# shenyunhang/APE

Hardware: NVIDIA H100
Metric: images_per_sec (higher is better)
Workload: dtype f16

## Files before the change

ape_b200/csrc/gemm_tc.cu:

```cuda
#include <stdlib.h>

#include <type_traits>

#include "common.cuh"
#include "tc.cuh"

namespace ape {
namespace {

constexpr int BM = 128, BK = 64, WG_K = 16;
constexpr int kConsumerWarps = 8;
constexpr int kThreads = 32 * kConsumerWarps + 32;

enum Act { ACT_NONE = 0, ACT_RELU = 1, ACT_GELU = 2, ACT_SWIGLU = 3, ACT_CLAMP = 4 };
enum Res { RES_NONE = 0, RES_F32 = 1, RES_16 = 2 };

template <bool OUT32, int ACT, int RES, bool LN = false, bool ROPE = false, bool STATS = false>
struct Epi {
  static constexpr bool out32 = OUT32, ln = LN, rope = ROPE, stats = STATS;
  static constexpr int act = ACT, res = RES;
};

struct GemmParams {
  void *C;
// ... 245 lines not shown
  if (threadIdx.x == 0) trace_stamp(p, 1);

  if (warp == kConsumerWarps) {
    if (lane == 0) {
      uint32_t stage = 0, phase = 0;
      int m_blk, n_blk;
      for (int t = 0; tile_at(t, m_blk, n_blk); ++t) {
        for (int kb = 0; kb < p.k_blocks; ++kb) {
          tc::mbar_wait(&s.empty[stage], phase ^ 1);
          tc::mbar_expect_tx(&s.full[stage], STAGE_BYTES);
          if (p.conv) {
            const int img = m_blk / p.conv_tiles_img, tt = m_blk - img * p.conv_tiles_img;
            const int ty = tt / p.conv_tiles_x, tx = tt - ty * p.conv_tiles_x;
            const int tap = kb / p.conv_cblks, cb = kb - tap * p.conv_cblks;
            tc::tma_load_4d(s.a[stage], &map_a, &s.full[stage], cb * BK, tx * p.conv_tw + tap % 3 - 1, ty * p.conv_th + tap / 3 - 1, img);
          } else {
            tc::tma_load_2d(s.a[stage], &map_a, &s.full[stage], kb * BK, m_blk * BM);
          }
          if (CL == 1) {
            tc::tma_load_2d(s.b[stage], &map_b, &s.full[stage], kb * BK, n_blk * BN);
          } else {
            constexpr int HALF_ROWS = BN / CL;
            tc::tma_load_2d_multicast(s.b[stage] + rank * HALF_ROWS * BK * 2, &map_b, &s.full[stage], kb * BK,
                                      n_blk * BN + rank * HALF_ROWS, (uint16_t)((1u << CL) - 1));
          }
          if (++stage == STAGES) { stage = 0; phase ^= 1; }
        }
      }
    }
    __syncwarp();
  } else {
    const int wg = warp / 4;
    float acc[BN / 2];
#pragma unroll
    for (int i = 0; i < BN / 2; ++i) acc[i] = 0.f;
    auto release = [&](uint32_t st) {
      if (lane == 0) {
        tc::mbar_arrive(&s.empty[st]);
        if (CL > 1) tc::mbar_arrive_cluster(tc::mapa_u32(&s.empty[st], (uint32_t)(rank ^ 1)));
      }
    };
    uint32_t stage = 0, phase = 0;
    int m_blk, n_blk;
    for (int t = 0; tile_at(t, m_blk, n_blk); ++t) {
      uint32_t prev = 0;
      for (int kb = 0; kb < p.k_blocks; ++kb) {
        tc::mbar_wait(&s.full[stage], phase);
        if (kb == 0 && t == 0 && threadIdx.x == 0) trace_stamp(p, 2);
        const uint64_t da = tc::make_smem_desc_sw128(tc::smem_u32(s.a[stage] + wg * 64 * BK * 2));
        const uint64_t db = tc::make_smem_desc_sw128(tc::smem_u32(s.b[stage]));
        tc::fence_regs<BN / 2>(acc);
        tc::wgmma_fence();
#pragma unroll
        for (int k = 0; k < BK / WG_K; ++k)
          tc::Wgmma<BN, TI>::template ss<0>(acc, da + 2 * k, db + 2 * k, (kb | k) != 0);
        tc::wgmma_commit();
        tc::fence_regs<BN / 2>(acc);
        if (kb > 0) {
          tc::wgmma_wait<1>();
          release(prev);
        }
        prev = stage;
        if (++stage == STAGES) { stage = 0; phase ^= 1; }
      }
      tc::wgmma_wait<0>();
      tc::fence_regs<BN / 2>(acc);
      release(prev);
      if (threadIdx.x == 0) {
        trace_stamp(p, 3);
        if (t == 0) trace_stamp(p, 4);
        trace_stamp(p, 5);
      }
      if constexpr (kArgmax<E>) argmax_epilogue<BN>(p, acc, m_blk, n_blk, wg, lane);
      else if (!E::rope && p.fast && (m_blk + 1) * BM <= p.M && (n_blk + 1) * BN <= p.N) epilogue<E, TI, BN, true>(p, acc, m_blk, n_blk, wg, lane);
      else epilogue<E, TI, BN, false>(p, acc, m_blk, n_blk, wg, lane);
    }
    if (threadIdx.x == 0) trace_stamp(p, 6);
  }
  __syncthreads();
  if (CL > 1) tc::cluster_sync_all();
  if (threadIdx.x == 0) trace_stamp(p, 7);
}

typedef CUresult (*EncodeTiledFn)(CUtensorMap *, CUtensorMapDataType, cuuint32_t, void *, const cuuint64_t *,
                                  const cuuint64_t *, const cuuint32_t *, const cuuint32_t *, CUtensorMapInterleave,
                                  CUtensorMapSwizzle, CUtensorMapL2promotion, CUtensorMapFloatOOBfill);

EncodeTiledFn get_encoder() {
  static EncodeTiledFn fn = nullptr;
  if (fn == nullptr) {
    void *ptr = nullptr;
    cudaDriverEntryPointQueryResult qres;
    if (cudaGetDriverEntryPoint("cuTensorMapEncodeTiled", &ptr, cudaEnableDefault, &qres) == cudaSuccess &&
        qres == cudaDriverEntryPointSuccess)
      fn = reinterpret_cast<EncodeTiledFn>(ptr);
  }
  return fn;
}

int make_map(CUtensorMap *map, const void *base, int dtype, long long rows, long long K, long long ld, int box_rows,
             int box_cols = BK) {
  EncodeTiledFn enc = get_encoder();
  if (!enc) return fail(APE_ERR_UNSUPPORTED, "gemm: cuTensorMapEncodeTiled not available from the driver");
  cuuint64_t dims[2] = {(cuuint64_t)K, (cuuint64_t)rows};
  cuuint64_t strides[1] = {(cuuint64_t)ld * (dtype == APE_DTYPE_F32 ? 4 : 2)};
  cuuint32_t box[2] = {(cuuint32_t)box_cols, (cuuint32_t)box_rows};
  cuuint32_t estr[2] = {1, 1};
  CUresult r = enc(map, dtype == APE_DTYPE_F32 ? CU_TENSOR_MAP_DATA_TYPE_FLOAT32
                        : dtype == APE_DTYPE_F16 ? CU_TENSOR_MAP_DATA_TYPE_FLOAT16 : CU_TENSOR_MAP_DATA_TYPE_BFLOAT16, 2,
                   const_cast<void *>(base), dims, strides, box, estr, CU_TENSOR_MAP_INTERLEAVE_NONE,
                   CU_TENSOR_MAP_SWIZZLE_128B, CU_TENSOR_MAP_L2_PROMOTION_L2_256B, CU_TENSOR_MAP_FLOAT_OOB_FILL_NONE);
  if (r != CUDA_SUCCESS) return fail(APE_ERR_INVALID_ARG, "gemm: cuTensorMapEncodeTiled failed (%d)", (int)r);
  return APE_OK;
}

int num_sms() {
  static int n = 0;
  if (n == 0) {
    int dev = 0;
    cudaGetDevice(&dev);
    cudaDeviceGetAttribute(&n, cudaDevAttrMultiProcessorCount, dev);
    if (n <= 0) n = 132;
  }
  return n;
}

template <int BN, int STAGES, int CL, typename TI, class E>
int launch_gemm(const CUtensorMap &ma, const CUtensorMap &mb, GemmParams &p, cudaStream_t st) {
  using Smem = GemmSmem<BN, STAGES>;
  const size_t smem = sizeof(Smem) + 1024;
  auto k = gemm_tc_kernel<BN, STAGES, CL, TI, E>;
  static bool attr_set = false;
  if (!attr_set) {
    cudaError_t e = cudaFuncSetAttribute(k, cudaFuncAttributeMaxDynamicSharedMemorySize, (int)smem);
    if (e != cudaSuccess) return fail((int)e, "gemm: cudaFuncSetAttribute(smem=%zu): %s", smem, cudaGetErrorString(e));
    attr_set = true;
  }
  p.n_blocks = (p.N + BN - 1) / BN;
  const int m_groups = (p.m_blocks + CL - 1) / CL;
  const int groups = m_groups * p.n_blocks;
  const int max_clusters = num_sms() / CL;
  const int clusters = groups < max_clusters ? groups : max_clusters;
  p.band = std::min(m_groups, (clusters + p.n_blocks - 1) / p.n_blocks);
  cudaLaunchConfig_t cfg{};
  cfg.gridDim = dim3((unsigned)(clusters * CL));
  cfg.blockDim = dim3(kThreads);
  cfg.dynamicSmemBytes = smem;
  cfg.stream = st;
  cudaLaunchAttribute attr[2];
  attr[0].id = cudaLaunchAttributeClusterDimension;
  attr[0].val.clusterDim.x = CL;
  attr[0].val.clusterDim.y = 1;
  attr[0].val.clusterDim.z = 1;
  attr[1].id = cudaLaunchAttributeProgrammaticStreamSerialization;
  attr[1].val.programmaticStreamSerializationAllowed = pdl_enabled() ? 1 : 0;
  cfg.attrs = attr;
  cfg.numAttrs = 2;
  cudaError_t e = cudaLaunchKernelEx(&cfg, k, ma, mb, p);
  if (e != cudaSuccess) return fail((int)e, "gemm_tc_kernel launch: %s", cudaGetErrorString(e));
  return check_launch("gemm_tc_kernel");
}

template <int CL, typename TI, class E>
int launch_bn(int bn, const CUtensorMap &ma, const CUtensorMap &mb, GemmParams &p, cudaStream_t st) {
  if (bn == 256) return launch_gemm<256, 4, CL, TI, E>(ma, mb, p, st);
  return launch_gemm<128, 6, CL, TI, E>(ma, mb, p, st);
}

struct EpiKey {
  bool out32;
  int act, res;
  bool ln, rope, stats;
};

#define APE_GEMM_EPILOGUES(X)                                                                                            \
  X(false, ACT_NONE, RES_NONE, false, false, false) X(false, ACT_RELU, RES_NONE, false, false, false)                   \
  X(false, ACT_GELU, RES_NONE, false, false, false) X(false, ACT_NONE, RES_F32, false, false, false)                    \
  X(false, ACT_NONE, RES_16, false, false, false) X(false, ACT_RELU, RES_16, false, false, false)                       \
  X(false, ACT_GELU, RES_16, false, false, false) X(false, ACT_SWIGLU, RES_NONE, false, false, false)                   \
  X(false, ACT_SWIGLU, RES_NONE, false, false, true) X(false, ACT_NONE, RES_NONE, false, true, false)                   \
  X(true, ACT_NONE, RES_NONE, false, false, false) X(true, ACT_RELU, RES_NONE, false, false, false)                     \
  X(true, ACT_GELU, RES_NONE, false, false, false) X(true, ACT_SWIGLU, RES_NONE, false, false, false)                   \
  X(true, ACT_CLAMP, RES_NONE, false, false, false) X(true, ACT_NONE, RES_F32, false, false, false)                     \
  X(true, ACT_NONE, RES_16, false, false, false) X(true, ACT_NONE, RES_F32, true, false, false)

template <int CL, typename TI>
int launch_epi(int bn, const EpiKey &k, const CUtensorMap &ma, const CUtensorMap &mb, GemmParams &p, cudaStream_t st) {
#define APE_EPI_CASE(o, a, r, l, ro, s)                                                                                  \
  if (k.out32 == o && k.act == a && k.res == r && k.ln == l && k.rope == ro && k.stats == s)                           \
    return launch_bn<CL, TI, Epi<o, a, r, l, ro, s>>(bn, ma, mb, p, st);
  APE_GEMM_EPILOGUES(APE_EPI_CASE)
#undef APE_EPI_CASE
  return fail(APE_ERR_UNSUPPORTED, "gemm: no kernel for the epilogue (fp32 out %d, act %d, residual %d, ln %d, rope %d, stats %d)",
              (int)k.out32, k.act, k.res, (int)k.ln, (int)k.rope, (int)k.stats);
}

int launch_any(int bn, bool cluster, int in_dtype, const EpiKey &k, const CUtensorMap &ma, const CUtensorMap &mb, GemmParams &p,
               cudaStream_t st) {
  if (in_dtype == APE_DTYPE_BF16)
    return cluster ? launch_epi<2, __nv_bfloat16>(bn, k, ma, mb, p, st) : launch_epi<1, __nv_bfloat16>(bn, k, ma, mb, p, st);
  return cluster ? launch_epi<2, __half>(bn, k, ma, mb, p, st) : launch_epi<1, __half>(bn, k, ma, mb, p, st);
}

}
}

using namespace ape;

struct RopeArgs {
  const float *cos, *sin;
  const int *pos;
  int cols, npos;
};

struct FuseArgs {
  const float *ln_part, *ln_colsum;
  int ln_nparts;
  float ln_inv_c, ln_eps;
  float *stats_out;
  int stats_nslab;
};

static long long *g_gemm_trace = nullptr;

extern "C" void ape_gemm_set_trace(long long *device_buffer) { g_gemm_trace = device_buffer; }

static int gemm_impl(const void *A, int64_t lda, const void *W, int64_t ldw, void *C, int64_t ldc,
                     const float *bias, const void *residual, int64_t ldr, int res_dtype, int M, int N, int K, int in_dtype,
                     int out_dtype, int act, int tile_n, const RopeArgs *rope, void *stream, const FuseArgs *fuse = nullptr) {
  if (residual && res_dtype != APE_DTYPE_F32 && res_dtype != APE_DTYPE_F16 && res_dtype != APE_DTYPE_BF16)
    return fail(APE_ERR_INVALID_ARG, "gemm: bad res_dtype %d", res_dtype);
  if (in_dtype != APE_DTYPE_F16 && in_dtype != APE_DTYPE_BF16)
    return fail(APE_ERR_INVALID_ARG, "gemm: operands must be fp16 or bf16 (got dtype %d)", in_dtype);
  if (out_dtype != APE_DTYPE_F32 && out_dtype != APE_DTYPE_F16 && out_dtype != APE_DTYPE_BF16)
    return fail(APE_ERR_INVALID_ARG, "gemm: bad out_dtype %d", out_dtype);
  if (act < 0 || act > ACT_CLAMP) return fail(APE_ERR_INVALID_ARG, "gemm: bad activation %d", act);
  if (M < 0 || N <= 0 || K <= 0) return fail(APE_ERR_INVALID_ARG, "gemm: bad sizes M=%d N=%d K=%d", M, N, K);
  if (M == 0) return APE_OK;
  if (!A || !W || !C) return fail(APE_ERR_NULL_PTR, "gemm: null pointer argument");
  if ((lda * 2) % 16 || (ldw * 2) % 16 || (reinterpret_cast<uintptr_t>(A) & 15) || (reinterpret_cast<uintptr_t>(W) & 15))
    return fail(APE_ERR_INVALID_ARG, "gemm: A/W base and row pitch must be 16-byte aligned (TMA)");
  if (lda < K || ldw < K) return fail(APE_ERR_INVALID_ARG, "gemm: row pitch smaller than K");
  if (act == ACT_SWIGLU && ((N & 1) || residual)) return fail(APE_ERR_INVALID_ARG, "gemm: swiglu needs even N, no residual");
  const int bn = (tile_n & 0xfff) > 0 ? (tile_n & 0xfff) : 128;
  if (bn != 128 && bn != 256) return fail(APE_ERR_INVALID_ARG, "gemm: tile_n must be 128 or 256");
  if (tile_n & 0x2000) return fail(APE_ERR_UNSUPPORTED, "gemm: tile_n flag 0x2000 (CTA-pair MMA) is not available on sm_90a");
  cudaStream_t st = reinterpret_cast<cudaStream_t>(stream);
  const int m_blocks = (M + BM - 1) / BM;
  const bool cluster = m_blocks >= 2 && (tile_n & 0x1000) == 0 && ((tile_n & 0x4000) != 0 || K >= 2048);
  CUtensorMap ma, mb;
  if (int rc = make_map(&ma, A, in_dtype, M, K, lda, BM)) return rc;
  if (int rc = make_map(&mb, W, in_dtype, N, K, ldw, cluster ? bn / 2 : bn)) return rc;
  GemmParams p{};
  p.C = C; p.bias = bias; p.residual = residual; p.ldc = ldc; p.ldr = ldr;
  p.M = M; p.N = N; p.K = K;
  p.m_blocks = m_blocks;
  p.k_blocks = (K + BK - 1) / BK;
  p.trace = g_gemm_trace;
  const int oe = out_dtype == APE_DTYPE_F32 ? 4 : 2;
  if (oe == 2 && out_dtype != in_dtype)
    return fail(APE_ERR_UNSUPPORTED, "gemm: a 16-bit output must have the operand dtype (out %d, operands %d)", out_dtype, in_dtype);
  if (residual && res_dtype != APE_DTYPE_F32 && res_dtype != in_dtype)
    return fail(APE_ERR_UNSUPPORTED, "gemm: a 16-bit residual must have the operand dtype (residual %d, operands %d)", res_dtype, in_dtype);
  const auto pairs = [](const void *ptr, long long ld, int esize) {
    return (ld % 2) == 0 && (reinterpret_cast<uintptr_t>(ptr) % (2 * esize)) == 0;
  };
  p.vec_out = pairs(C, ldc, oe);
  p.fast = p.vec_out && (!residual || pairs(residual, ldr, res_dtype == APE_DTYPE_F32 ? 4 : 2)) &&
           reinterpret_cast<uintptr_t>(bias) % 8 == 0 && (!fuse || reinterpret_cast<uintptr_t>(fuse->ln_colsum) % 8 == 0);
  EpiKey key{oe == 4, act, !residual ? RES_NONE : res_dtype == APE_DTYPE_F32 ? RES_F32 : RES_16, false, rope != nullptr, false};
  const int n_out = act == ACT_SWIGLU ? N / 2 : N;
  if (fuse) {
    if (fuse->ln_part) {
      if (out_dtype != APE_DTYPE_F32 || !fuse->ln_colsum || fuse->ln_nparts <= 0 || act == ACT_SWIGLU)
        return fail(APE_ERR_INVALID_ARG, "gemm+ln: needs an fp32 output, column sums and partial statistics");
      p.ln_part = fuse->ln_part; p.ln_colsum = fuse->ln_colsum; p.ln_nparts = fuse->ln_nparts;
      p.ln_inv_c = fuse->ln_inv_c; p.ln_eps = fuse->ln_eps;
      key.ln = true;
    }
    if (fuse->stats_out) {
      if (oe != 2 || act != ACT_SWIGLU || fuse->stats_nslab != (n_out + 63) / 64)
        return fail(APE_ERR_INVALID_ARG, "gemm+stats: needs the SwiGLU epilogue with a 16-bit output and stats_nslab = ceil(N/2/64)");
      p.stats_out = fuse->stats_out; p.stats_nslab = fuse->stats_nslab;
      key.stats = true;
    }
  }
  if (rope) {
    if (oe != 2 || act != ACT_NONE || rope->cols % 64 != 0 || rope->cols > N || rope->npos <= 0 || !rope->cos || !rope->sin)
      return fail(APE_ERR_INVALID_ARG, "gemm+rope: needs a 16-bit output, no activation, rope_cols a multiple of 64 <= N");
    p.rope_cos = rope->cos; p.rope_sin = rope->sin; p.rope_pos = rope->pos; p.rope_cols = rope->cols; p.rope_npos = rope->npos;
  }
  return launch_any(bn, cluster, in_dtype, key, ma, mb, p, st);
}

extern "C" int ape_gemm_tn(const void *A, int64_t lda, const void *W, int64_t ldw, void *C, int64_t ldc,
                           const float *bias, const void *residual, int64_t ldr, int M, int N, int K, int in_dtype,
                           int out_dtype, int act, int tile_n, void *stream) {
  return gemm_impl(A, lda, W, ldw, C, ldc, bias, residual, ldr, out_dtype, M, N, K, in_dtype, out_dtype, act, tile_n, nullptr,
                   stream);
}

extern "C" int ape_gemm_tn_ex(const void *A, int64_t lda, const void *W, int64_t ldw, void *C, int64_t ldc,
                              const float *bias, const void *residual, int64_t ldr, int res_dtype, int M, int N, int K,
                              int in_dtype, int out_dtype, int act, int tile_n, void *stream) {
  return gemm_impl(A, lda, W, ldw, C, ldc, bias, residual, ldr, res_dtype, M, N, K, in_dtype, out_dtype, act, tile_n, nullptr,
                   stream);
}

extern "C" int ape_gemm_tn_fused(const void *A, int64_t lda, const void *W, int64_t ldw, void *C, int64_t ldc, const float *bias,
                                 const void *residual, int64_t ldr, int res_dtype, int M, int N, int K, int in_dtype, int out_dtype,
                                 int act, int tile_n, const float *ln_part, int ln_nparts, const float *ln_colsum, float ln_inv_c,
                                 float ln_eps, float *stats_out, int stats_nslab, void *stream) {
  FuseArgs f{ln_part, ln_colsum, ln_nparts, ln_inv_c, ln_eps, stats_out, stats_nslab};
  return gemm_impl(A, lda, W, ldw, C, ldc, bias, residual, ldr, res_dtype, M, N, K, in_dtype, out_dtype, act, tile_n, nullptr,
                   stream, &f);
}

static int make_map_nhwc(CUtensorMap *map, const void *base, int dtype, int B, int H, int W, int C, int bw, int bh) {
  EncodeTiledFn enc = get_encoder();
  if (!enc) return fail(APE_ERR_UNSUPPORTED, "conv: cuTensorMapEncodeTiled not available from the driver");
  cuuint64_t dims[4] = {(cuuint64_t)C, (cuuint64_t)W, (cuuint64_t)H, (cuuint64_t)B};
  cuuint64_t strides[3] = {(cuuint64_t)C * 2, (cuuint64_t)W * C * 2, (cuuint64_t)H * W * C * 2};
  cuuint32_t box[4] = {64, (cuuint32_t)bw, (cuuint32_t)bh, 1};
  cuuint32_t estr[4] = {1, 1, 1, 1};
  CUresult r = enc(map, dtype == APE_DTYPE_F16 ? CU_TENSOR_MAP_DATA_TYPE_FLOAT16 : CU_TENSOR_MAP_DATA_TYPE_BFLOAT16, 4,
                   const_cast<void *>(base), dims, strides, box, estr, CU_TENSOR_MAP_INTERLEAVE_NONE,
                   CU_TENSOR_MAP_SWIZZLE_128B, CU_TENSOR_MAP_L2_PROMOTION_L2_256B, CU_TENSOR_MAP_FLOAT_OOB_FILL_NONE);
  if (r != CUDA_SUCCESS) return fail(APE_ERR_INVALID_ARG, "conv: cuTensorMapEncodeTiled failed (%d)", (int)r);
  return APE_OK;
}

extern "C" int ape_conv3x3_nhwc(const void *x, const void *w, void *y, const float *bias, int B, int H, int W, int Cin, int Cout,
                                int dtype, int act, void *stream) {
  if (dtype != APE_DTYPE_F16 && dtype != APE_DTYPE_BF16) return fail(APE_ERR_INVALID_ARG, "conv3x3: fp16 / bf16 only");
  if (B <= 0 || H <= 0 || W <= 0 || Cin <= 0 || Cout <= 0) return fail(APE_ERR_INVALID_ARG, "conv3x3: bad sizes");
  if (Cin % 64 || Cout % 8) return fail(APE_ERR_UNSUPPORTED, "conv3x3: Cin must be a multiple of 64 and Cout of 8 (got %d, %d)", Cin, Cout);
  if (act != ACT_NONE && act != ACT_RELU && act != ACT_GELU) return fail(APE_ERR_INVALID_ARG, "conv3x3: activation %d", act);
  int tw = 128;
  while (tw > 8 && W % tw) tw >>= 1;
  const int th = 128 / tw;
  if (W % tw || H % th) return fail(APE_ERR_UNSUPPORTED, "conv3x3: %dx%d image is not a whole number of %dx%d pixel tiles", H, W, th, tw);
  if (!x || !w || !y) return fail(APE_ERR_NULL_PTR, "conv3x3: null pointer argument");
  if ((reinterpret_cast<uintptr_t>(x) | reinterpret_cast<uintptr_t>(w) | reinterpret_cast<uintptr_t>(y)) & 15)
    return fail(APE_ERR_INVALID_ARG, "conv3x3: tensors must be 16-byte aligned");
  const int K = 9 * Cin, M = B * H * W, N = Cout;
  const int bn = 128;
  const int m_blocks = M / BM;
  const bool cluster = m_blocks >= 2 && m_blocks % 2 == 0;
  CUtensorMap ma, mb;
  if (int rc = make_map_nhwc(&ma, x, dtype, B, H, W, Cin, tw, th)) return rc;
  if (int rc = make_map(&mb, w, dtype, N, K, K, cluster ? bn / 2 : bn)) return rc;
  GemmParams p{};
  p.C = y; p.bias = bias; p.ldc = N; p.M = M; p.N = N; p.K = K;
  p.m_blocks = m_blocks;
  p.k_blocks = K / BK;
  p.vec_out = 1;
  p.fast = reinterpret_cast<uintptr_t>(bias) % 8 == 0;
  p.conv = 1; p.conv_tw = tw; p.conv_th = th; p.conv_tiles_x = W / tw; p.conv_tiles_img = (W / tw) * (H / th); p.conv_cblks = Cin / 64;
  p.conv_W = W; p.conv_H = H;
  const EpiKey key{false, act, RES_NONE, false, false, false};
  return launch_any(bn, cluster, dtype, key, ma, mb, p, reinterpret_cast<cudaStream_t>(stream));
}

extern "C" int ape_gemm_tn_argmax(const void *A, int64_t lda, const void *W, int64_t ldw, uint64_t *keys, int M, int N, int K,
                                  int col_base, int in_dtype, void *stream) {
  if (in_dtype != APE_DTYPE_F16 && in_dtype != APE_DTYPE_BF16)
    return fail(APE_ERR_INVALID_ARG, "gemm_argmax: operands must be fp16 or bf16 (got dtype %d)", in_dtype);
  if (M < 0 || N <= 0 || K <= 0 || col_base < 0 || (long long)col_base + N > 0x7fffffffLL)
    return fail(APE_ERR_INVALID_ARG, "gemm_argmax: bad sizes M=%d N=%d K=%d col_base=%d", M, N, K, col_base);
  if (M == 0) return APE_OK;
  if (!A || !W || !keys) return fail(APE_ERR_NULL_PTR, "gemm_argmax: null pointer argument");
  if ((lda * 2) % 16 || (ldw * 2) % 16 || (reinterpret_cast<uintptr_t>(A) & 15) || (reinterpret_cast<uintptr_t>(W) & 15))
    return fail(APE_ERR_INVALID_ARG, "gemm_argmax: A/W base and row pitch must be 16-byte aligned (TMA)");
  if (lda < K || ldw < K) return fail(APE_ERR_INVALID_ARG, "gemm_argmax: row pitch smaller than K");
  if (reinterpret_cast<uintptr_t>(keys) & 7) return fail(APE_ERR_INVALID_ARG, "gemm_argmax: keys must be 8-byte aligned");
  constexpr int bn = 128;
  CUtensorMap ma, mb;
  if (int rc = make_map(&ma, A, in_dtype, M, K, lda, BM)) return rc;
  if (int rc = make_map(&mb, W, in_dtype, N, K, ldw, bn)) return rc;
  GemmParams p{};
  p.C = keys; p.M = M; p.N = N; p.K = K;
  p.m_blocks = (M + BM - 1) / BM;
  p.k_blocks = (K + BK - 1) / BK;
  p.trace = g_gemm_trace;
  p.argmax_col_base = col_base;
  cudaStream_t st = reinterpret_cast<cudaStream_t>(stream);
  if (in_dtype == APE_DTYPE_BF16) return launch_gemm<bn, 6, 1, __nv_bfloat16, EpiArgmax>(ma, mb, p, st);
  return launch_gemm<bn, 6, 1, __half, EpiArgmax>(ma, mb, p, st);
}

extern "C" int ape_gemm_tn_rope(const void *A, int64_t lda, const void *W, int64_t ldw, void *C, int64_t ldc,
                                const float *bias, int M, int N, int K, int in_dtype, int out_dtype, const float *cos_table,
                                const float *sin_table, const int *pos_map, int npos, int head_dim, int rope_cols,
                                int tile_n, void *stream) {
  if (head_dim != 64) return fail(APE_ERR_UNSUPPORTED, "gemm+rope: head_dim %d (only 64)", head_dim);
  if ((reinterpret_cast<uintptr_t>(cos_table) | reinterpret_cast<uintptr_t>(sin_table)) & 15)
    return fail(APE_ERR_INVALID_ARG, "gemm+rope: cos / sin tables must be 16-byte aligned");
  RopeArgs r{cos_table, sin_table, pos_map, rope_cols, npos};
  return gemm_impl(A, lda, W, ldw, C, ldc, bias, nullptr, 0, out_dtype, M, N, K, in_dtype, out_dtype, ACT_NONE, tile_n, &r, stream);
}
```

ape_b200/csrc/tc.cuh:

```cuda
#pragma once
#include <cuda.h>
#include <cuda_runtime.h>
#include <cuda_fp16.h>
#include <cuda_bf16.h>
#include <stdint.h>

namespace ape {
namespace tc {

__device__ __forceinline__ uint32_t smem_u32(const void *p) {
  return (uint32_t)__cvta_generic_to_shared(p);
}

__device__ __forceinline__ void mbar_init(uint64_t *bar, uint32_t count) {
  asm volatile("mbarrier.init.shared::cta.b64 [%0], %1;" ::"r"(smem_u32(bar)), "r"(count) : "memory");
}
__device__ __forceinline__ void fence_mbar_init() {
  asm volatile("fence.mbarrier_init.release.cluster;" ::: "memory");
}
__device__ __forceinline__ void mbar_expect_tx(uint64_t *bar, uint32_t bytes) {
  asm volatile("mbarrier.arrive.expect_tx.shared::cta.b64 _, [%0], %1;" ::"r"(smem_u32(bar)), "r"(bytes)
               : "memory");
}
__device__ __forceinline__ void mbar_arrive(uint64_t *bar) {
  asm volatile("mbarrier.arrive.shared::cta.b64 _, [%0];" ::"r"(smem_u32(bar)) : "memory");
}
__device__ __forceinline__ void mbar_wait(uint64_t *bar, uint32_t parity) {
  const uint32_t addr = smem_u32(bar);
  for (uint32_t it = 0; it < (1u << 26); ++it) {
    uint32_t done;
    asm volatile(
        "{\n\t.reg .pred p;\n\t"
        "mbarrier.try_wait.parity.shared::cta.b64 p, [%1], %2;\n\t"
        "selp.u32 %0, 1, 0, p;\n\t}"
        : "=r"(done)
        : "r"(addr), "r"(parity)
        : "memory");
    if (done) return;
  }
  __trap();
}

__device__ __forceinline__ void prefetch_tensormap(const CUtensorMap *m) {
  asm volatile("prefetch.tensormap [%0];" ::"l"(m) : "memory");
}
__device__ __forceinline__ void tma_load_2d(void *smem_dst, const CUtensorMap *map, uint64_t *bar, int c0, int c1) {
  asm volatile(
      "cp.async.bulk.tensor.2d.shared::cluster.global.tile.mbarrier::complete_tx::bytes [%0], [%1, {%3, %4}], [%2];"
      ::"r"(smem_u32(smem_dst)), "l"(map), "r"(smem_u32(bar)), "r"(c0), "r"(c1)
      : "memory");
}

__device__ __forceinline__ void tma_load_4d(void *smem_dst, const CUtensorMap *map, uint64_t *bar, int c0, int c1, int c2, int c3) {
  asm volatile(
      "cp.async.bulk.tensor.4d.shared::cluster.global.tile.mbarrier::complete_tx::bytes [%0], [%1, {%3, %4, %5, %6}], [%2];"
      ::"r"(smem_u32(smem_dst)), "l"(map), "r"(smem_u32(bar)), "r"(c0), "r"(c1), "r"(c2), "r"(c3)
      : "memory");
}

__device__ __forceinline__ void tma_load_2d_multicast(void *smem_dst, const CUtensorMap *map, uint64_t *bar, int c0,
                                                      int c1, uint16_t cta_mask) {
  asm volatile(
      "cp.async.bulk.tensor.2d.shared::cluster.global.tile.mbarrier::complete_tx::bytes.multicast::cluster"
      " [%0], [%1, {%3, %4}], [%2], %5;"
      ::"r"(smem_u32(smem_dst)), "l"(map), "r"(smem_u32(bar)), "r"(c0), "r"(c1), "h"(cta_mask)
      : "memory");
}
__device__ __forceinline__ uint32_t cluster_ctarank() {
  uint32_t r;
  asm volatile("mov.u32 %0, %%cluster_ctarank;" : "=r"(r));
  return r;
}
__device__ __forceinline__ void cluster_sync_all() {
  asm volatile("barrier.cluster.arrive.release.aligned;" ::: "memory");
  asm volatile("barrier.cluster.wait.acquire.aligned;" ::: "memory");
}

__device__ __forceinline__ uint32_t mapa_u32(const void *p, uint32_t rank) {
  uint32_t r;
  asm volatile("mapa.shared::cluster.u32 %0, %1, %2;" : "=r"(r) : "r"(smem_u32(p)), "r"(rank));
  return r;
}
__device__ __forceinline__ void mbar_arrive_cluster(uint32_t bar_cluster_addr) {
  asm volatile("mbarrier.arrive.release.cluster.shared::cluster.b64 _, [%0];" ::"r"(bar_cluster_addr) : "memory");
}

template <int N>
__device__ __forceinline__ void setmaxnreg_inc() { asm volatile("setmaxnreg.inc.sync.aligned.u32 %0;" ::"n"(N)); }
template <int N>
__device__ __forceinline__ void setmaxnreg_dec() { asm volatile("setmaxnreg.dec.sync.aligned.u32 %0;" ::"n"(N)); }

__device__ __forceinline__ void wgmma_fence() { asm volatile("wgmma.fence.sync.aligned;" ::: "memory"); }
__device__ __forceinline__ void wgmma_commit() { asm volatile("wgmma.commit_group.sync.aligned;" ::: "memory"); }
template <int N>
__device__ __forceinline__ void wgmma_wait() { asm volatile("wgmma.wait_group.sync.aligned %0;" ::"n"(N) : "memory"); }
template <int N>
__device__ __forceinline__ void fence_regs(float *r) {
#pragma unroll
  for (int i = 0; i < N; ++i) asm volatile("" : "+f"(r[i])::"memory");
}
__device__ __forceinline__ void fence_proxy_async() { asm volatile("fence.proxy.async.shared::cta;" ::: "memory"); }

__device__ __forceinline__ uint64_t make_smem_desc_sw128(uint32_t smem_addr) {
  uint64_t d = 0;
  d |= (uint64_t)((smem_addr & 0x3FFFF) >> 4);
  d |= (uint64_t)1 << 16;
  d |= (uint64_t)(1024 >> 4) << 32;
  d |= (uint64_t)1 << 62;
  return d;
}

template <int N, typename T>
struct Wgmma;
template <> struct Wgmma<64, __half> {
  template <int TRANS_B>
  __device__ static __forceinline__ void ss(float *d, uint64_t da, uint64_t db, int scale_d) {
    asm volatile(
        "{\n.reg .pred p;\nsetp.ne.b32 p, %34, 0;\n"
        "wgmma.mma_async.sync.aligned.m64n64k16.f32.f16.f16 {%0, %1, %2, %3, %4, %5, %6, %7, %8, %9, %10, %11, %12, %13, %14, %15, %16, %17, %18, %19, %20, %21, %22, %23, %24, %25, %26, %27, %28, %29, %30, %31}, %32, %33, p, 1, 1, 0, %35;\n}\n"
        : "+f"(d[0]), "+f"(d[1]), "+f"(d[2]), "+f"(d[3]), "+f"(d[4]), "+f"(d[5]), "+f"(d[6]), "+f"(d[7]), "+f"(d[8]), "+f"(d[9]), "+f"(d[10]), "+f"(d[11]), "+f"(d[12]), "+f"(d[13]), "+f"(d[14]), "+f"(d[15]), "+f"(d[16]), "+f"(d[17]), "+f"(d[18]), "+f"(d[19]), "+f"(d[20]), "+f"(d[21]), "+f"(d[22]), "+f"(d[23]), "+f"(d[24]), "+f"(d[25]), "+f"(d[26]), "+f"(d[27]), "+f"(d[28]), "+f"(d[29]), "+f"(d[30]), "+f"(d[31])
        : "l"(da), "l"(db), "r"(scale_d), "n"(TRANS_B));
  }
  template <int TRANS_B>
  __device__ static __forceinline__ void rs(float *d, const uint32_t *a, uint64_t db, int scale_d) {
    asm volatile(
        "{\n.reg .pred p;\nsetp.ne.b32 p, %37, 0;\n"
        "wgmma.mma_async.sync.aligned.m64n64k16.f32.f16.f16 {%0, %1, %2, %3, %4, %5, %6, %7, %8, %9, %10, %11, %12, %13, %14, %15, %16, %17, %18, %19, %20, %21, %22, %23, %24, %25, %26, %27, %28, %29, %30, %31}, {%32, %33, %34, %35}, %36, p, 1, 1, %38;\n}\n"
        : "+f"(d[0]), "+f"(d[1]), "+f"(d[2]), "+f"(d[3]), "+f"(d[4]), "+f"(d[5]), "+f"(d[6]), "+f"(d[7]), "+f"(d[8]), "+f"(d[9]), "+f"(d[10]), "+f"(d[11]), "+f"(d[12]), "+f"(d[13]), "+f"(d[14]), "+f"(d[15]), "+f"(d[16]), "+f"(d[17]), "+f"(d[18]), "+f"(d[19]), "+f"(d[20]), "+f"(d[21]), "+f"(d[22]), "+f"(d[23]), "+f"(d[24]), "+f"(d[25]), "+f"(d[26]), "+f"(d[27]), "+f"(d[28]), "+f"(d[29]), "+f"(d[30]), "+f"(d[31])
        : "r"(a[0]), "r"(a[1]), "r"(a[2]), "r"(a[3]), "l"(db), "r"(scale_d), "n"(TRANS_B));
  }
};
template <> struct Wgmma<64, __nv_bfloat16> {
  template <int TRANS_B>
  __device__ static __forceinline__ void ss(float *d, uint64_t da, uint64_t db, int scale_d) {
    asm volatile(
        "{\n.reg .pred p;\nsetp.ne.b32 p, %34, 0;\n"
        "wgmma.mma_async.sync.aligned.m64n64k16.f32.bf16.bf16 {%0, %1, %2, %3, %4, %5, %6, %7, %8, %9, %10, %11, %12, %13, %14, %15, %16, %17, %18, %19, %20, %21, %22, %23, %24, %25, %26, %27, %28, %29, %30, %31}, %32, %33, p, 1, 1, 0, %35;\n}\n"
        : "+f"(d[0]), "+f"(d[1]), "+f"(d[2]), "+f"(d[3]), "+f"(d[4]), "+f"(d[5]), "+f"(d[6]), "+f"(d[7]), "+f"(d[8]), "+f"(d[9]), "+f"(d[10]), "+f"(d[11]), "+f"(d[12]), "+f"(d[13]), "+f"(d[14]), "+f"(d[15]), "+f"(d[16]), "+f"(d[17]), "+f"(d[18]), "+f"(d[19]), "+f"(d[20]), "+f"(d[21]), "+f"(d[22]), "+f"(d[23]), "+f"(d[24]), "+f"(d[25]), "+f"(d[26]), "+f"(d[27]), "+f"(d[28]), "+f"(d[29]), "+f"(d[30]), "+f"(d[31])
        : "l"(da), "l"(db), "r"(scale_d), "n"(TRANS_B));
  }
  template <int TRANS_B>
  __device__ static __forceinline__ void rs(float *d, const uint32_t *a, uint64_t db, int scale_d) {
    asm volatile(
        "{\n.reg .pred p;\nsetp.ne.b32 p, %37, 0;\n"
        "wgmma.mma_async.sync.aligned.m64n64k16.f32.bf16.bf16 {%0, %1, %2, %3, %4, %5, %6, %7, %8, %9, %10, %11, %12, %13, %14, %15, %16, %17, %18, %19, %20, %21, %22, %23, %24, %25, %26, %27, %28, %29, %30, %31}, {%32, %33, %34, %35}, %36, p, 1, 1, %38;\n}\n"
        : "+f"(d[0]), "+f"(d[1]), "+f"(d[2]), "+f"(d[3]), "+f"(d[4]), "+f"(d[5]), "+f"(d[6]), "+f"(d[7]), "+f"(d[8]), "+f"(d[9]), "+f"(d[10]), "+f"(d[11]), "+f"(d[12]), "+f"(d[13]), "+f"(d[14]), "+f"(d[15]), "+f"(d[16]), "+f"(d[17]), "+f"(d[18]), "+f"(d[19]), "+f"(d[20]), "+f"(d[21]), "+f"(d[22]), "+f"(d[23]), "+f"(d[24]), "+f"(d[25]), "+f"(d[26]), "+f"(d[27]), "+f"(d[28]), "+f"(d[29]), "+f"(d[30]), "+f"(d[31])
        : "r"(a[0]), "r"(a[1]), "r"(a[2]), "r"(a[3]), "l"(db), "r"(scale_d), "n"(TRANS_B));
  }
};
template <> struct Wgmma<128, __half> {
  template <int TRANS_B>
  __device__ static __forceinline__ void ss(float *d, uint64_t da, uint64_t db, int scale_d) {
    asm volatile(
        "{\n.reg .pred p;\nsetp.ne.b32 p, %66, 0;\n"
        "wgmma.mma_async.sync.aligned.m64n128k16.f32.f16.f16 {%0, %1, %2, %3, %4, %5, %6, %7, %8, %9, %10, %11, %12, %13, %14, %15, %16, %17, %18, %19, %20, %21, %22, %23, %24, %25, %26, %27, %28, %29, %30, %31, %32, %33, %34, %35, %36, %37, %38, %39, %40, %41, %42, %43, %44, %45, %46, %47, %48, %49, %50, %51, %52, %53, %54, %55, %56, %57, %58, %59, %60, %61, %62, %63}, %64, %65, p, 1, 1, 0, %67;\n}\n"
        : "+f"(d[0]), "+f"(d[1]), "+f"(d[2]), "+f"(d[3]), "+f"(d[4]), "+f"(d[5]), "+f"(d[6]), "+f"(d[7]), "+f"(d[8]), "+f"(d[9]), "+f"(d[10]), "+f"(d[11]), "+f"(d[12]), "+f"(d[13]), "+f"(d[14]), "+f"(d[15]), "+f"(d[16]), "+f"(d[17]), "+f"(d[18]), "+f"(d[19]), "+f"(d[20]), "+f"(d[21]), "+f"(d[22]), "+f"(d[23]), "+f"(d[24]), "+f"(d[25]), "+f"(d[26]), "+f"(d[27]), "+f"(d[28]), "+f"(d[29]), "+f"(d[30]), "+f"(d[31]), "+f"(d[32]), "+f"(d[33]), "+f"(d[34]), "+f"(d[35]), "+f"(d[36]), "+f"(d[37]), "+f"(d[38]), "+f"(d[39]), "+f"(d[40]), "+f"(d[41]), "+f"(d[42]), "+f"(d[43]), "+f"(d[44]), "+f"(d[45]), "+f"(d[46]), "+f"(d[47]), "+f"(d[48]), "+f"(d[49]), "+f"(d[50]), "+f"(d[51]), "+f"(d[52]), "+f"(d[53]), "+f"(d[54]), "+f"(d[55]), "+f"(d[56]), "+f"(d[57]), "+f"(d[58]), "+f"(d[59]), "+f"(d[60]), "+f"(d[61]), "+f"(d[62]), "+f"(d[63])
        : "l"(da), "l"(db), "r"(scale_d), "n"(TRANS_B));
  }
  template <int TRANS_B>
  __device__ static __forceinline__ void rs(float *d, const uint32_t *a, uint64_t db, int scale_d) {
    asm volatile(
        "{\n.reg .pred p;\nsetp.ne.b32 p, %69, 0;\n"
        "wgmma.mma_async.sync.aligned.m64n128k16.f32.f16.f16 {%0, %1, %2, %3, %4, %5, %6, %7, %8, %9, %10, %11, %12, %13, %14, %15, %16, %17, %18, %19, %20, %21, %22, %23, %24, %25, %26, %27, %28, %29, %30, %31, %32, %33, %34, %35, %36, %37, %38, %39, %40, %41, %42, %43, %44, %45, %46, %47, %48, %49, %50, %51, %52, %53, %54, %55, %56, %57, %58, %59, %60, %61, %62, %63}, {%64, %65, %66, %67}, %68, p, 1, 1, %70;\n}\n"
        : "+f"(d[0]), "+f"(d[1]), "+f"(d[2]), "+f"(d[3]), "+f"(d[4]), "+f"(d[5]), "+f"(d[6]), "+f"(d[7]), "+f"(d[8]), "+f"(d[9]), "+f"(d[10]), "+f"(d[11]), "+f"(d[12]), "+f"(d[13]), "+f"(d[14]), "+f"(d[15]), "+f"(d[16]), "+f"(d[17]), "+f"(d[18]), "+f"(d[19]), "+f"(d[20]), "+f"(d[21]), "+f"(d[22]), "+f"(d[23]), "+f"(d[24]), "+f"(d[25]), "+f"(d[26]), "+f"(d[27]), "+f"(d[28]), "+f"(d[29]), "+f"(d[30]), "+f"(d[31]), "+f"(d[32]), "+f"(d[33]), "+f"(d[34]), "+f"(d[35]), "+f"(d[36]), "+f"(d[37]), "+f"(d[38]), "+f"(d[39]), "+f"(d[40]), "+f"(d[41]), "+f"(d[42]), "+f"(d[43]), "+f"(d[44]), "+f"(d[45]), "+f"(d[46]), "+f"(d[47]), "+f"(d[48]), "+f"(d[49]), "+f"(d[50]), "+f"(d[51]), "+f"(d[52]), "+f"(d[53]), "+f"(d[54]), "+f"(d[55]), "+f"(d[56]), "+f"(d[57]), "+f"(d[58]), "+f"(d[59]), "+f"(d[60]), "+f"(d[61]), "+f"(d[62]), "+f"(d[63])
        : "r"(a[0]), "r"(a[1]), "r"(a[2]), "r"(a[3]), "l"(db), "r"(scale_d), "n"(TRANS_B));
  }
};
template <> struct Wgmma<128, __nv_bfloat16> {
  template <int TRANS_B>
  __device__ static __forceinline__ void ss(float *d, uint64_t da, uint64_t db, int scale_d) {
    asm volatile(
        "{\n.reg .pred p;\nsetp.ne.b32 p, %66, 0;\n"
        "wgmma.mma_async.sync.aligned.m64n128k16.f32.bf16.bf16 {%0, %1, %2, %3, %4, %5, %6, %7, %8, %9, %10, %11, %12, %13, %14, %15, %16, %17, %18, %19, %20, %21, %22, %23, %24, %25, %26, %27, %28, %29, %30, %31, %32, %33, %34, %35, %36, %37, %38, %39, %40, %41, %42, %43, %44, %45, %46, %47, %48, %49, %50, %51, %52, %53, %54, %55, %56, %57, %58, %59, %60, %61, %62, %63}, %64, %65, p, 1, 1, 0, %67;\n}\n"
        : "+f"(d[0]), "+f"(d[1]), "+f"(d[2]), "+f"(d[3]), "+f"(d[4]), "+f"(d[5]), "+f"(d[6]), "+f"(d[7]), "+f"(d[8]), "+f"(d[9]), "+f"(d[10]), "+f"(d[11]), "+f"(d[12]), "+f"(d[13]), "+f"(d[14]), "+f"(d[15]), "+f"(d[16]), "+f"(d[17]), "+f"(d[18]), "+f"(d[19]), "+f"(d[20]), "+f"(d[21]), "+f"(d[22]), "+f"(d[23]), "+f"(d[24]), "+f"(d[25]), "+f"(d[26]), "+f"(d[27]), "+f"(d[28]), "+f"(d[29]), "+f"(d[30]), "+f"(d[31]), "+f"(d[32]), "+f"(d[33]), "+f"(d[34]), "+f"(d[35]), "+f"(d[36]), "+f"(d[37]), "+f"(d[38]), "+f"(d[39]), "+f"(d[40]), "+f"(d[41]), "+f"(d[42]), "+f"(d[43]), "+f"(d[44]), "+f"(d[45]), "+f"(d[46]), "+f"(d[47]), "+f"(d[48]), "+f"(d[49]), "+f"(d[50]), "+f"(d[51]), "+f"(d[52]), "+f"(d[53]), "+f"(d[54]), "+f"(d[55]), "+f"(d[56]), "+f"(d[57]), "+f"(d[58]), "+f"(d[59]), "+f"(d[60]), "+f"(d[61]), "+f"(d[62]), "+f"(d[63])
// ... 52 lines not shown
```

Baseline: 34.21.

## Add ping-pong warpgroup GEMM kernel for large tile counts

Adds a ping-pong variant of the wgmma GEMM. Each of two consumer warpgroups owns a whole 128x128 tile, and the two alternate their mainloop through named barriers so one group's epilogue overlaps the other's MMA. It is picked automatically when the tile count is at least twice the SM count, with no cluster and tile width 128, and it is also used for the argmax GEMM. The cost is more producer threads and one warpgroup holding 128 accumulators, which adds register pressure and a new ordering scheme between the groups.

```diff
diff --git a/ape_b200/csrc/gemm_tc.cu b/ape_b200/csrc/gemm_tc.cu
--- a/ape_b200/csrc/gemm_tc.cu
+++ b/ape_b200/csrc/gemm_tc.cu
@@ -351,6 +351,126 @@
   if (threadIdx.x == 0) trace_stamp(p, 7);
 }
 
+constexpr int kPpThreads = 32 * kConsumerWarps + 128;
+constexpr int kOrderBar = 1;
+
+template <typename TI, class E>
+__global__ void __launch_bounds__(kPpThreads, 1)
+gemm_pp_kernel(const __grid_constant__ CUtensorMap map_a, const __grid_constant__ CUtensorMap map_b, const GemmParams p) {
+  constexpr int BN = 128, STAGES = 6;
+  extern __shared__ uint8_t smem_raw[];
+  pdl_launch_dependents();
+  if (threadIdx.x == 0) trace_stamp(p, 0);
+  using Smem = GemmSmem<BN, STAGES>;
+  Smem &s = *reinterpret_cast<Smem *>((reinterpret_cast<uintptr_t>(smem_raw) + 1023) & ~uintptr_t(1023));
+  constexpr uint32_t STAGE_BYTES = (BM + BN) * BK * 2;
+
+  const int warp = threadIdx.x / 32, lane = threadIdx.x % 32;
+  const int num_tiles = p.m_blocks * p.n_blocks;
+  auto tile_at = [&](int t, int &m_blk, int &n_blk) -> bool {
+    const int tile = blockIdx.x + t * gridDim.x;
+    if (tile >= num_tiles) return false;
+    const int per_band = p.band * p.n_blocks;
+    const int band = tile / per_band, r = tile - band * per_band;
+    const int rows = min(p.band, p.m_blocks - band * p.band);
+    n_blk = r / rows;
+    m_blk = band * p.band + r - n_blk * rows;
+    return true;
+  };
+
+  if (warp == kConsumerWarps && lane == 0) {
+    tc::prefetch_tensormap(&map_a);
+    tc::prefetch_tensormap(&map_b);
+#pragma unroll
+    for (int i = 0; i < STAGES; ++i) {
+      tc::mbar_init(&s.full[i], 1);
+      tc::mbar_init(&s.empty[i], 4);
+    }
+    tc::fence_mbar_init();
+  }
+  __syncthreads();
+  pdl_wait();
+  if (threadIdx.x == 0) trace_stamp(p, 1);
+
+  if (warp >= kConsumerWarps) {
+    tc::setmaxnreg_dec<40>();
+    if (warp == kConsumerWarps && lane == 0) {
+      uint32_t stage = 0, phase = 0;
+      int m_blk, n_blk;
+      for (int t = 0; tile_at(t, m_blk, n_blk); ++t) {
+        for (int kb = 0; kb < p.k_blocks; ++kb) {
+          tc::mbar_wait(&s.empty[stage], phase ^ 1);
+          tc::mbar_expect_tx(&s.full[stage], STAGE_BYTES);
+          tc::tma_load_2d(s.a[stage], &map_a, &s.full[stage], kb * BK, m_blk * BM);
+          tc::tma_load_2d(s.b[stage], &map_b, &s.full[stage], kb * BK, n_blk * BN);
+          if (++stage == STAGES) { stage = 0; phase ^= 1; }
+        }
+      }
+    }
+    __syncwarp();
+  } else {
+    tc::setmaxnreg_inc<232>();
+    const int wg = warp / 4;
+    float acc[BN];
+#pragma unroll
+    for (int i = 0; i < BN; ++i) acc[i] = 0.f;
+    auto release = [&](uint32_t st) {
+      if (lane == 0) tc::mbar_arrive(&s.empty[st]);
+    };
+    int m_blk, n_blk;
+    for (int t = wg; tile_at(t, m_blk, n_blk); t += 2) {
+      if (t > 0) tc::named_bar_sync(kOrderBar + wg, 256);
+      const uint32_t g0 = (uint32_t)t * p.k_blocks;
+      uint32_t stage = g0 % STAGES, phase = (g0 / STAGES) & 1, prev = 0;
+      for (int kb = 0; kb < p.k_blocks; ++kb) {
+        tc::mbar_wait(&s.full[stage], phase);
+        if (kb == 0 && t == 0 && threadIdx.x == 0) trace_stamp(p, 2);
+        const uint64_t da = tc::make_smem_desc_sw128(tc::smem_u32(s.a[stage]));
+        const uint64_t da_hi = tc::make_smem_desc_sw128(tc::smem_u32(s.a[stage] + 64 * BK * 2));
+        const uint64_t db = tc::make_smem_desc_sw128(tc::smem_u32(s.b[stage]));
+        tc::fence_regs<BN>(acc);
+        tc::wgmma_fence();
+#pragma unroll
+        for (int k = 0; k < BK / WG_K; ++k) {
+          tc::Wgmma<BN, TI>::template ss<0>(acc, da + 2 * k, db + 2 * k, (kb | k) != 0);
+          tc::Wgmma<BN, TI>::template ss<0>(acc + 64, da_hi + 2 * k, db + 2 * k, (kb | k) != 0);
+        }
+        tc::wgmma_commit();
+        tc::fence_regs<BN>(acc);
+        if (kb > 0) {
+          tc::wgmma_wait<1>();
+          release(prev);
+        }
+        prev = stage;
+        if (++stage == STAGES) { stage = 0; phase ^= 1; }
+      }
+      int m_nx, n_nx;
+      if (tile_at(t + 1, m_nx, n_nx)) tc::named_bar_arrive(kOrderBar + (wg ^ 1), 256);
+      tc::wgmma_wait<0>();
+      tc::fence_regs<BN>(acc);
+      release(prev);
+      if (threadIdx.x == 0) {
+        trace_stamp(p, 3);
+        if (t == 0) trace_stamp(p, 4);
+        trace_stamp(p, 5);
+      }
+      if constexpr (kArgmax<E>) {
+        argmax_epilogue<BN>(p, acc, m_blk, n_blk, 0, lane);
+        argmax_epilogue<BN>(p, acc + 64, m_blk, n_blk, 1, lane);
+      } else if (!E::rope && p.fast && (m_blk + 1) * BM <= p.M && (n_blk + 1) * BN <= p.N) {
+        epilogue<E, TI, BN, true>(p, acc, m_blk, n_blk, 0, lane);
+        epilogue<E, TI, BN, true>(p, acc + 64, m_blk, n_blk, 1, lane);
+      } else {
+        epilogue<E, TI, BN, false>(p, acc, m_blk, n_blk, 0, lane);
+        epilogue<E, TI, BN, false>(p, acc + 64, m_blk, n_blk, 1, lane);
+      }
+    }
+    if (threadIdx.x == 0) trace_stamp(p, 6);
+  }
+  __syncthreads();
+  if (threadIdx.x == 0) trace_stamp(p, 7);
+}
+
 typedef CUresult (*EncodeTiledFn)(CUtensorMap *, CUtensorMapDataType, cuuint32_t, void *, const cuuint64_t *,
                                   const cuuint64_t *, const cuuint32_t *, const cuuint32_t *, CUtensorMapInterleave,
                                   CUtensorMapSwizzle, CUtensorMapL2promotion, CUtensorMapFloatOOBfill);
@@ -394,11 +514,12 @@
   return n;
 }
 
-template <int BN, int STAGES, int CL, typename TI, class E>
+template <int BN, int STAGES, int CL, typename TI, class E, bool PP = false>
 int launch_gemm(const CUtensorMap &ma, const CUtensorMap &mb, GemmParams &p, cudaStream_t st) {
+  static_assert(!PP || (BN == 128 && STAGES == 6 && CL == 1), "gemm_pp_kernel is BN = 128, 6 stages, single CTA");
   using Smem = GemmSmem<BN, STAGES>;
   const size_t smem = sizeof(Smem) + 1024;
-  auto k = gemm_tc_kernel<BN, STAGES, CL, TI, E>;
+  auto k = PP ? gemm_pp_kernel<TI, E> : gemm_tc_kernel<BN, STAGES, CL, TI, E>;
   static bool attr_set = false;
   if (!attr_set) {
     cudaError_t e = cudaFuncSetAttribute(k, cudaFuncAttributeMaxDynamicSharedMemorySize, (int)smem);
@@ -413,7 +534,7 @@
   p.band = std::min(m_groups, (clusters + p.n_blocks - 1) / p.n_blocks);
   cudaLaunchConfig_t cfg{};
   cfg.gridDim = dim3((unsigned)(clusters * CL));
-  cfg.blockDim = dim3(kThreads);
+  cfg.blockDim = dim3(PP ? kPpThreads : kThreads);
   cfg.dynamicSmemBytes = smem;
   cfg.stream = st;
   cudaLaunchAttribute attr[2];
@@ -431,8 +552,10 @@
 }
 
 template <int CL, typename TI, class E>
-int launch_bn(int bn, const CUtensorMap &ma, const CUtensorMap &mb, GemmParams &p, cudaStream_t st) {
+int launch_bn(int bn, bool pp, const CUtensorMap &ma, const CUtensorMap &mb, GemmParams &p, cudaStream_t st) {
   if (bn == 256) return launch_gemm<256, 4, CL, TI, E>(ma, mb, p, st);
+  if constexpr (CL == 1)
+    if (pp) return launch_gemm<128, 6, 1, TI, E, true>(ma, mb, p, st);
   return launch_gemm<128, 6, CL, TI, E>(ma, mb, p, st);
 }
 
@@ -454,22 +577,24 @@
   X(true, ACT_NONE, RES_16, false, false, false) X(true, ACT_NONE, RES_F32, true, false, false)
 
 template <int CL, typename TI>
-int launch_epi(int bn, const EpiKey &k, const CUtensorMap &ma, const CUtensorMap &mb, GemmParams &p, cudaStream_t st) {
+int launch_epi(int bn, bool pp, const EpiKey &k, const CUtensorMap &ma, const CUtensorMap &mb, GemmParams &p, cudaStream_t st) {
 #define APE_EPI_CASE(o, a, r, l, ro, s)                                                                                  \
   if (k.out32 == o && k.act == a && k.res == r && k.ln == l && k.rope == ro && k.stats == s)                           \
-    return launch_bn<CL, TI, Epi<o, a, r, l, ro, s>>(bn, ma, mb, p, st);
+    return launch_bn<CL, TI, Epi<o, a, r, l, ro, s>>(bn, pp, ma, mb, p, st);
   APE_GEMM_EPILOGUES(APE_EPI_CASE)
 #undef APE_EPI_CASE
   return fail(APE_ERR_UNSUPPORTED, "gemm: no kernel for the epilogue (fp32 out %d, act %d, residual %d, ln %d, rope %d, stats %d)",
               (int)k.out32, k.act, k.res, (int)k.ln, (int)k.rope, (int)k.stats);
 }
 
-int launch_any(int bn, bool cluster, int in_dtype, const EpiKey &k, const CUtensorMap &ma, const CUtensorMap &mb, GemmParams &p,
-               cudaStream_t st) {
+int launch_any(int bn, bool cluster, bool pp, int in_dtype, const EpiKey &k, const CUtensorMap &ma, const CUtensorMap &mb,
+               GemmParams &p, cudaStream_t st) {
   if (in_dtype == APE_DTYPE_BF16)
-    return cluster ? launch_epi<2, __nv_bfloat16>(bn, k, ma, mb, p, st) : launch_epi<1, __nv_bfloat16>(bn, k, ma, mb, p, st);
-  return cluster ? launch_epi<2, __half>(bn, k, ma, mb, p, st) : launch_epi<1, __half>(bn, k, ma, mb, p, st);
-}
+    return cluster ? launch_epi<2, __nv_bfloat16>(bn, false, k, ma, mb, p, st) : launch_epi<1, __nv_bfloat16>(bn, pp, k, ma, mb, p, st);
+  return cluster ? launch_epi<2, __half>(bn, false, k, ma, mb, p, st) : launch_epi<1, __half>(bn, pp, k, ma, mb, p, st);
+}
+
+bool use_pingpong(int tiles) { return tiles >= 2 * num_sms(); }
 
 }
 }
@@ -515,8 +640,12 @@
   if (bn != 128 && bn != 256) return fail(APE_ERR_INVALID_ARG, "gemm: tile_n must be 128 or 256");
   if (tile_n & 0x2000) return fail(APE_ERR_UNSUPPORTED, "gemm: tile_n flag 0x2000 (CTA-pair MMA) is not available on sm_90a");
   cudaStream_t st = reinterpret_cast<cudaStream_t>(stream);
+  const bool force_pp = (tile_n & 0x8000) != 0, force_coop = (tile_n & 0x10000) != 0;
+  if (force_pp && (force_coop || bn != 128 || (tile_n & 0x4000)))
+    return fail(APE_ERR_INVALID_ARG, "gemm: tile_n flag 0x8000 (ping-pong) needs tile width 128, no cluster and no 0x10000");
   const int m_blocks = (M + BM - 1) / BM;
-  const bool cluster = m_blocks >= 2 && (tile_n & 0x1000) == 0 && ((tile_n & 0x4000) != 0 || K >= 2048);
+  const bool cluster = m_blocks >= 2 && !force_pp && (tile_n & 0x1000) == 0 && ((tile_n & 0x4000) != 0 || K >= 2048);
+  const bool pp = !cluster && bn == 128 && !force_coop && (force_pp || use_pingpong(m_blocks * ((N + bn - 1) / bn)));
   CUtensorMap ma, mb;
   if (int rc = make_map(&ma, A, in_dtype, M, K, lda, BM)) return rc;
   if (int rc = make_map(&mb, W, in_dtype, N, K, ldw, cluster ? bn / 2 : bn)) return rc;
@@ -559,7 +688,7 @@
       return fail(APE_ERR_INVALID_ARG, "gemm+rope: needs a 16-bit output, no activation, rope_cols a multiple of 64 <= N");
     p.rope_cos = rope->cos; p.rope_sin = rope->sin; p.rope_pos = rope->pos; p.rope_cols = rope->cols; p.rope_npos = rope->npos;
   }
-  return launch_any(bn, cluster, in_dtype, key, ma, mb, p, st);
+  return launch_any(bn, cluster, pp, in_dtype, key, ma, mb, p, st);
 }
 
 extern "C" int ape_gemm_tn(const void *A, int64_t lda, const void *W, int64_t ldw, void *C, int64_t ldc,
@@ -628,7 +757,7 @@
   p.conv = 1; p.conv_tw = tw; p.conv_th = th; p.conv_tiles_x = W / tw; p.conv_tiles_img = (W / tw) * (H / th); p.conv_cblks = Cin / 64;
   p.conv_W = W; p.conv_H = H;
   const EpiKey key{false, act, RES_NONE, false, false, false};
-  return launch_any(bn, cluster, dtype, key, ma, mb, p, reinterpret_cast<cudaStream_t>(stream));
+  return launch_any(bn, cluster, false, dtype, key, ma, mb, p, reinterpret_cast<cudaStream_t>(stream));
 }
 
 extern "C" int ape_gemm_tn_argmax(const void *A, int64_t lda, const void *W, int64_t ldw, uint64_t *keys, int M, int N, int K,
@@ -654,6 +783,10 @@
   p.trace = g_gemm_trace;
   p.argmax_col_base = col_base;
   cudaStream_t st = reinterpret_cast<cudaStream_t>(stream);
+  if (use_pingpong(p.m_blocks * ((N + bn - 1) / bn))) {
+    if (in_dtype == APE_DTYPE_BF16) return launch_gemm<bn, 6, 1, __nv_bfloat16, EpiArgmax, true>(ma, mb, p, st);
+    return launch_gemm<bn, 6, 1, __half, EpiArgmax, true>(ma, mb, p, st);
+  }
   if (in_dtype == APE_DTYPE_BF16) return launch_gemm<bn, 6, 1, __nv_bfloat16, EpiArgmax>(ma, mb, p, st);
   return launch_gemm<bn, 6, 1, __half, EpiArgmax>(ma, mb, p, st);
 }
diff --git a/ape_b200/csrc/tc.cuh b/ape_b200/csrc/tc.cuh
--- a/ape_b200/csrc/tc.cuh
+++ b/ape_b200/csrc/tc.cuh
@@ -90,6 +90,13 @@
 template <int N>
 __device__ __forceinline__ void setmaxnreg_dec() { asm volatile("setmaxnreg.dec.sync.aligned.u32 %0;" ::"n"(N)); }
 
+__device__ __forceinline__ void named_bar_sync(int id, int threads) {
+  asm volatile("bar.sync %0, %1;" ::"r"(id), "r"(threads) : "memory");
+}
+__device__ __forceinline__ void named_bar_arrive(int id, int threads) {
+  asm volatile("bar.arrive %0, %1;" ::"r"(id), "r"(threads) : "memory");
+}
+
 __device__ __forceinline__ void wgmma_fence() { asm volatile("wgmma.fence.sync.aligned;" ::: "memory"); }
 __device__ __forceinline__ void wgmma_commit() { asm volatile("wgmma.commit_group.sync.aligned;" ::: "memory"); }
 template <int N>
```

After: 35.64, median of 6. 1.04x the previous value.
